# ImIntheMiddle/EmLoco

Measured on AMD Instinct MI355X. Metric: env-steps/sec (SMPL humanoid, num_envs), higher is better.
Workload: dtype f32

## Files before the change

### emloco_amd/csrc/emloco_types.h

```cpp
#pragma once
#define EMLOCO_PART_WORDS 416
#include "../../include/emloco_sim.h"
#define EMLOCO_PART_TAG(seq, part) ((seq) * 4u + (unsigned)(part))
#define EMLOCO_ERR_PART_TIMEOUT 1u

#define EMLOCO_TOPO_PARENT 0
#define EMLOCO_TOPO_DEPTH 24
#define EMLOCO_TOPO_CHILD 48
#define EMLOCO_TOPO_PDPACK 120
#define EMLOCO_TOPO_CAND 144
#define EMLOCO_TOPO_SCPAIR 240
#define EMLOCO_TOPO_WORDS 560

#define EMLOCO_MB_DYN 0
#define EMLOCO_MB_GEO 384
#define EMLOCO_MB_CAP 576
#define EMLOCO_MB_DRV 832
#define EMLOCO_MODEL_WORDS 1112

struct EmlocoSimDev {
    int n_env, n_cand, max_depth, sc_n;
    int sc_nseg;
    const int *topo;
    const float *model;
// ... 7 lines not shown
    const unsigned char *hf_mv;
    long long *prof;
    const long long *step_skip;
    const int *step_ids;
    int n_slots;
    const int *step_order;
    unsigned *step_ticks;
    int n_parts; unsigned part_seq;
    float *part_state;
    unsigned *part_flag;
    unsigned *err;
    int part_spin_max;
    int part_poison;
    unsigned long long *step_start;
};
```

### emloco_amd/csrc/sim_capi.hip

```cpp
#include <hip/hip_runtime.h>
#include <cstdlib>
#include <cstdio>
#include <cstring>
#include <string>
#include <vector>
#ifdef EMLOCO_SIM_PAIR
#include "sim_pair_kernels.hip"
#define EMLOCO_SIM_ENVS_PER_WG 2
#else
#include "sim_kernels.hip"
#define EMLOCO_SIM_ENVS_PER_WG 1
#endif
#include "topology.h"
#include "model_pack.h"
#include "sim_state.h"

namespace {

thread_local std::string g_err;

int fail(int code, const char *what, hipError_t e = hipSuccess) {
    char buf[512];
    if (e != hipSuccess) snprintf(buf, sizeof(buf), "%s: %s", what, hipGetErrorString(e));
    else snprintf(buf, sizeof(buf), "%s", what);
// ... 276 lines not shown
    if (!s || !dev_forces) return fail(EMLOCO_E_ARG, "emloco_sim_set_dof_actuation_force: null argument");
    if (!s->prepared) return fail(EMLOCO_E_STATE, "emloco_sim_set_dof_actuation_force: sim not prepared");
    if (dev_forces != s->d_tgt.p)
        HIPCHK(hipMemcpyAsync(s->d_tgt.p, dev_forces, (size_t)s->n_env * EMLOCO_NDOF * 4, hipMemcpyDeviceToDevice, (hipStream_t)stream));
    s->prm.drive_mode = 1;
    return EMLOCO_OK;
}

static int launch_order(EmlocoSim *s, hipStream_t st) {
    if (s->order_ready) { s->order_ready = false; return EMLOCO_OK; }
    hipLaunchKernelGGL(emloco::sim_order_kernel, dim3(1), dim3(1024), 0, st, s->d_ticks.p, s->n_env, s->d_order.p, s->d_order_ws.p);
    HIPCHK(hipGetLastError());
    return EMLOCO_OK;
}

int emloco_sim_step(EmlocoSim *s, int n_calls, void *stream) {
    if (!s) return fail(EMLOCO_E_ARG, "emloco_sim_step: null sim");
    if (!s->prepared) return fail(EMLOCO_E_STATE, "emloco_sim_step: sim not prepared");
    if (n_calls < 1) return fail(EMLOCO_E_ARG, "emloco_sim_step: n_calls < 1");
    if (const int rc = check_device_error(s, "emloco_sim_step")) return rc;
    EmlocoSimParams p = s->prm;
    p.n_sub = s->prm.n_sub * n_calls;
    hipStream_t st = (hipStream_t)stream;
    EmlocoSimDev d = s->dev;
    if (s->cost_order) {
        const int rc = launch_order(s, st);
        if (rc != EMLOCO_OK) return rc;
        d.step_order = s->d_order.p;
        d.step_ticks = s->d_ticks.p;
    }
    const int slot = s->ev_head;
    const bool timed = s->timing && (s->launch_no++ % s->timing_stride) == 0;
    if (timed) HIPCHK(hipEventRecord(s->ev0[slot], st));
    d.n_parts = s->n_parts < p.n_sub ? s->n_parts : p.n_sub;
    d.part_seq = ++s->part_seq; d.part_state = s->d_part_state.p; d.part_flag = s->d_part_flag.p;
    d.part_spin_max = s->part_spin_max; d.part_poison = s->part_poison;
    d.n_slots = s->n_env;
    const unsigned grid = (unsigned)(((s->n_env + EMLOCO_SIM_ENVS_PER_WG - 1) / EMLOCO_SIM_ENVS_PER_WG) * d.n_parts);
    if (d.hf) hipLaunchKernelGGL(emloco::sim_step_kernel<1>, dim3(grid), dim3(64), (size_t)s->lds_pad, st, p, d);
    else hipLaunchKernelGGL(emloco::sim_step_kernel<0>, dim3(grid), dim3(64), (size_t)s->lds_pad, st, p, d);
    HIPCHK(hipGetLastError());
    if (timed) {
        HIPCHK(hipEventRecord(s->ev1[slot], st));
        s->ev_head = (slot + 1) % EmlocoSim::kRing;
        if (s->ev_count < EmlocoSim::kRing) ++s->ev_count;
    }
    return EMLOCO_OK;
}

int emloco_sim_step_subset(EmlocoSim *s, int n_calls, const int64_t *dev_skip, const int32_t *dev_ids, int n_ids, void *stream) {
    if (!s) return fail(EMLOCO_E_ARG, "emloco_sim_step_subset: null sim");
    if (!s->prepared) return fail(EMLOCO_E_STATE, "emloco_sim_step_subset: sim not prepared");
    if (n_calls < 1) return fail(EMLOCO_E_ARG, "emloco_sim_step_subset: n_calls < 1");
    if ((dev_skip == nullptr) == (dev_ids == nullptr)) return fail(EMLOCO_E_ARG, "emloco_sim_step_subset: exactly one of skip flags / id list");
    if (dev_ids && (n_ids < 0 || n_ids > s->n_env)) return fail(EMLOCO_E_ARG, "emloco_sim_step_subset: bad id count");
    if (dev_ids && n_ids == 0) return EMLOCO_OK;
    if (const int rc = check_device_error(s, "emloco_sim_step_subset")) return rc;
    EmlocoSimParams p = s->prm;
    p.n_sub = s->prm.n_sub * n_calls;
    EmlocoSimDev d = s->dev;
    d.step_skip = (const long long *)dev_skip;
    d.step_ids = (const int *)dev_ids;
    hipStream_t st = (hipStream_t)stream;
    if (s->cost_order) {
        d.step_ticks = s->d_ticks.p;
        if (dev_skip) {
            const int rc = launch_order(s, st);
            if (rc != EMLOCO_OK) return rc;
            d.step_order = s->d_order.p;
        }
    }
    const bool timed = s->timing && dev_skip && (s->launch_no++ % s->timing_stride) == 0;
    const int slot = s->ev_head;
    if (timed) HIPCHK(hipEventRecord(s->ev0[slot], st));
    d.n_parts = dev_ids ? 1 : (s->n_parts < p.n_sub ? s->n_parts : p.n_sub);
    d.part_seq = ++s->part_seq; d.part_state = s->d_part_state.p; d.part_flag = s->d_part_flag.p;
    d.part_spin_max = s->part_spin_max; d.part_poison = s->part_poison;
    d.n_slots = dev_ids ? n_ids : s->n_env;
    const unsigned grid = (unsigned)(((d.n_slots + EMLOCO_SIM_ENVS_PER_WG - 1) / EMLOCO_SIM_ENVS_PER_WG) * d.n_parts);
    if (d.hf) hipLaunchKernelGGL(emloco::sim_step_kernel<1>, dim3(grid), dim3(64), (size_t)s->lds_pad, st, p, d);
    else hipLaunchKernelGGL(emloco::sim_step_kernel<0>, dim3(grid), dim3(64), (size_t)s->lds_pad, st, p, d);
    HIPCHK(hipGetLastError());
    if (timed) {
        HIPCHK(hipEventRecord(s->ev1[slot], st));
        s->ev_head = (slot + 1) % EmlocoSim::kRing;
        if (s->ev_count < EmlocoSim::kRing) ++s->ev_count;
    }
    return EMLOCO_OK;
}

int emloco_sim_set_split(EmlocoSim *s, int n_parts) {
    if (!s) return fail(EMLOCO_E_ARG, "emloco_sim_set_split: null sim");
    if (!s->prepared) return fail(EMLOCO_E_STATE, "emloco_sim_set_split: sim not prepared");
    if (n_parts < 1 || n_parts > 4) return fail(EMLOCO_E_ARG, "emloco_sim_set_split: 1 to 4 parts");
    if (n_parts > 1 && !s->d_part_state.p) {
        HIPCHK(hipSetDevice(s->device));
// ... 149 lines not shown
```

### emloco_amd/csrc/sim_kernels.hip

```cpp
#include <hip/hip_runtime.h>
#include "dev_math.h"
#include "sim_math.h"
#define cross3 fcross3
#define dot3 fdot3
#define dot6 fdot6
#define qmul fqmul
#define qnormalize fqnormalize
#define q2mat fq2mat
#define matvec3 fmatvec3
#define rotvec2quat frotvec2quat
#define quat2rotvec fquat2rotvec
#include "emloco_types.h"
#include "fk_device.h"
#include "order_device.h"

namespace emloco {

#define NB EMLOCO_NB
#define NDOF EMLOCO_NDOF
#define MAXC EMLOCO_MAXC
#define MAXR (3 * EMLOCO_MAXC)
#define MAXCAND EMLOCO_MAXCAND
#define EMLOCO_WH_MAX 1.0f
#define YLEN 30
// ... 197 lines not shown
                        if (dist > 1.0e-6f) { const float id_ = 1.0f / dist; for (int k = 0; k < 3; ++k) nsel[k] = dv[k] * id_; }
                        else for (int k = 0; k < 3; ++k) nsel[k] = fn[k] * ifn;
                    }
                } else if (side < 0.0f && face) {
                    const float dw = side * ifn;
                    if (dw > dsel) { dsel = dw; for (int k = 0; k < 3; ++k) nsel[k] = fn[k] * ifn; }
                }
            }
        }
    }
}

#ifndef EMLOCO_SIM_WAVES_PER_SIMD
#define EMLOCO_SIM_WAVES_PER_SIMD 3
#endif
template <int HF>
__device__ __forceinline__ void sim_step_env(const EmlocoSimParams &prm, const EmlocoSimDev &d, const int env, int &work, const int part, const int n_parts) {
    int lane = threadIdx.x;
    work = 0;

    enum { O_ROOT = 0, O_P = 16, O_V0 = 24, O_L = 36, O_PD = 48, O_R = O_PD + NB, O_W = O_R + NB * 12,
           O_L0 = O_W + NB * 24, O_CB = O_L0 + 44, O_CX = O_CB + MAXC / 4 + 3, O_CDIST = O_CX + 3 * MAXC, O_LAM = O_CDIST + MAXC,
           O_SLOT = O_LAM + MAXR, O_CRANGE = O_SLOT + 32, O_IA = O_CRANGE + 2 * NB / 4, O_G = O_IA + 180,
           O_PA = O_IA + NB * 24, O_A_ = O_PA + NB * 8, O_V = O_A_ + NB * 8,
           O_VF = O_V + NB * 8, O_AACC = O_VF + NB * 8, O_FEXT = O_AACC + NB * 8, O_PQ = O_FEXT + NB * 8,
           LDS_WORDS = (O_PQ + NB * 8 > O_G + MAXR * (MAXR + 1) / 2) ? O_PQ + NB * 8 : O_G + MAXR * (MAXR + 1) / 2 };
    static_assert(O_R % 4 == 0 && O_W % 4 == 0 && O_IA % 4 == 0 && O_PA % 4 == 0 && O_PQ % 4 == 0, "rows must be 16-byte aligned");
    static_assert(O_V - O_G >= EMLOCO_SC_MAXSEG * 8 + EMLOCO_SC_MAXHITS * 8 + 256, "limb-limb scratch does not fit its overlay");
    static_assert(LDS_WORDS * 4 <= 13312, "LDS per env above 160 KiB / 12 in 512-byte granules (three waves per SIMD, 12 envs per CU)");
    __shared__ __attribute__((aligned(16))) float lds[LDS_WORDS];
    float *sh_root = lds + O_ROOT;
    float *sh_V0 = lds + O_V0;
    float *sh_P = lds + O_P;
    float *sh_L = lds + O_L;
    int *sh_pd = (int *)(lds + O_PD);
    float (*sh_R)[12] = (float (*)[12])(lds + O_R);
    float (*sh_W)[24] = (float (*)[24])(lds + O_W);
    float *sh_L0 = lds + O_L0, *sh_L0i = lds + O_L0 + 36;
    unsigned char *sh_cbody = (unsigned char *)(lds + O_CB);
    float (*sh_cx)[3] = (float (*)[3])(lds + O_CX);
    float *sh_cdist = lds + O_CDIST;
    float *sh_lam = lds + O_LAM;
    signed char *sh_crange = (signed char *)(lds + O_CRANGE);
    unsigned char *sh_slot = (unsigned char *)(lds + O_SLOT);
// ... 19 lines not shown
    float *cf_env = d.contact_force + (size_t)env * NB * 3;
    float *lws_env = d.lambda_ws + (size_t)env * MAXCAND * 3;
    if (lane < NB) sh_pd[lane] = topo[EMLOCO_TOPO_PDPACK + lane];
    sh_slot[lane] = 255; sh_slot[lane + 64] = 255;

    const int sub_lo = (prm.n_sub * part) / n_parts, sub_hi = (prm.n_sub * (part + 1)) / n_parts;
    float *pst = d.part_state ? d.part_state + (long)env * EMLOCO_PART_WORDS : nullptr;
    float qj[4] = {0, 0, 0, 1}, wj[3] = {0, 0, 0}, edof[3] = {0, 0, 0};
    if (part == 0) {
        if ((lane < NB) && lane >= 1) {
            const float *ds = dofs_env + jdof * 2;
            float e[3] = {ds[0], ds[2], ds[4]};
            rotvec2quat(e, qj);
            wj[0] = ds[1]; wj[1] = ds[3]; wj[2] = ds[5];
            quat2rotvec(qj, edof);
        }
        if (lane == 0) {
            const float *rs = d.root_state + (long)env * 13;
            float q0[4] = {rs[3], rs[4], rs[5], rs[6]};
            qnormalize(q0);
            for (int k = 0; k < 3; ++k) { sh_root[k] = rs[k]; sh_root[7 + k] = rs[10 + k]; sh_root[10 + k] = rs[7 + k]; }
            for (int k = 0; k < 4; ++k) sh_root[3 + k] = q0[k];
        }
    } else {
        if (lane == 0) {
            int spins = 0;
            const unsigned want = EMLOCO_PART_TAG(d.part_seq, part - 1);
            while (part_flag_get(d.part_flag + env) != want && ++spins < d.part_spin_max) __builtin_amdgcn_s_sleep(16);
            sh_V0[0] = spins < d.part_spin_max ? 1.0f : 0.0f;
            if (spins >= d.part_spin_max) part_err_raise(d.err, EMLOCO_ERR_PART_TIMEOUT);
// ... 316 lines not shown
                    const int bi = sh_hitb[hh * 2], bj = sh_hitb[hh * 2 + 1];
                    if (bi == lane) for (int k = 0; k < 6; ++k) fe[k] += sh_hitw[hh * 6 + k];
                    else if (bj == lane) for (int k = 0; k < 6; ++k) fe[k] -= sh_hitw[hh * 6 + k];
                }
                for (int k = 0; k < 6; ++k) sh_fext[lane][k] = fe[k];
            }
            __syncthreads();
        }

        PSTAMP(1);
        if ((lane < NB)) {
            for (int k = 0; k < 3; ++k) {
                float dr[4];
                ld4(mdl, o_drv + 4 * k, dr);
                const float kp = lane >= 1 ? dr[0] : 0.0f, kd = lane >= 1 ? dr[1] : 0.0f;
                const float arm = lane >= 1 ? dr[2] : 0.0f, tgt = lane >= 1 ? tgt_env[jdof + k] : 0.0f;
                const float e = tgt - edof[k];
                if (prm.drive_mode == 1) {
                    const float eff = lane >= 1 ? dr[3] : 0.0f;
                    sat[k] = 2; tau[k] = tgt > eff ? eff : (tgt < -eff ? -eff : tgt); dd[k] = arm;
                } else {
                    sat[k] = 0; tau[k] = kp * e - (kd + h * kp) * wj[k]; dd[k] = arm + h * kd + h * h * kp;
                }
            }
        }

        PSTAMP(2);
#if defined(EMLOCO_DUMMY_VALU) || defined(EMLOCO_DUMMY_LDS) || defined(EMLOCO_DUMMY_SALU)
        {
#ifdef EMLOCO_DUMMY_VALU
            float z0 = h, z1 = h + 1.0f, z2 = h + 2.0f, z3 = h + 3.0f;
// ... 642 lines not shown
                    cross3(arm, ip, t);
                }
                for (int k = 0; k < 3; ++k) tq[k] = wave_sum(t[k]);
            }
            if (lane == 0) for (int k = 0; k < 3; ++k) sh_L[k] = (sh_L[4 + k] + tq[k]) * damp;
        }
        PSTAMP(9);
        bool clamped = false;
        if ((lane < NB) && lane >= 1) {
            float wn[3];
            for (int k = 0; k < 3; ++k) {
                wn[k] = fmaf(h, qdd[k], wj[k]) + dq[k];
                if (last) {
                    float dr[4];
                    ld4(mdl, o_drv + 4 * k, dr);
                    const float kpk = dr[0], kdk = dr[1], tgk = tgt_env[jdof + k];
                    const float effk = dr[3];
                    float tq = sat[k] == 0 ? kpk * (tgk - edof[k] - h * wn[k]) - kdk * wn[k]
                             : (sat[k] == 2 ? tgk : (sat[k] > 0 ? effk : -effk));
                    tq = tq > effk ? effk : (tq < -effk ? -effk : tq);
                    d.dof_force[(size_t)env * NDOF + jdof + k] = tq;
                }
                wj[k] = wn[k] * damp;
            }
            const float nj = sqrtf(dot3(wj, wj));
            if (nj > prm.max_ang_vel) { const float sc = prm.max_ang_vel / nj; wj[0] *= sc; wj[1] *= sc; wj[2] *= sc; clamped = true; }
            float e[3] = {h * wj[0], h * wj[1], h * wj[2]}, dqt[4], qn[4];
            rotvec2quat(e, dqt);
            qmul(qj, dqt, qn); qnormalize(qn);
            for (int k = 0; k < 4; ++k) qj[k] = qn[k];
            quat2rotvec(qj, edof);
// ... 52 lines not shown
            for (int k = 0; k < 3; ++k) { ds[2 * k] = edof[k]; ds[2 * k + 1] = wj[k]; }
        }
    }
    if (lane == 0) {
        float *rs = d.root_state + (long)env * 13;
        for (int k = 0; k < 3; ++k) { rs[k] = sh_root[k]; rs[7 + k] = sh_root[10 + k]; rs[10 + k] = sh_root[7 + k]; }
        for (int k = 0; k < 4; ++k) rs[3 + k] = sh_root[3 + k];
    }
    for (int s = 0; s < 2; ++s) {
        const int c = lane + 64 * s;
        if (c < MAXCAND) {
            const int os = sh_slot[c];
            for (int k = 0; k < 3; ++k) lws_env[c * 3 + k] = os != 255 ? sh_lam[3 * os + k] : 0.0f;
        }
    }
}
#undef o_dyn
#undef jdof
#undef o_drv

template <int HF>
__global__ void __attribute__((amdgpu_flat_work_group_size(64, 64), amdgpu_waves_per_eu(EMLOCO_SIM_WAVES_PER_SIMD, EMLOCO_SIM_WAVES_PER_SIMD)))
sim_step_kernel(EmlocoSimParams prm, EmlocoSimDev d) {
    const int n_parts = d.n_parts > 1 ? d.n_parts : 1;
    const int part = (int)blockIdx.x / d.n_env, slot = (int)blockIdx.x - part * d.n_env;
    if (part >= n_parts) return;
    int env = d.step_order ? d.step_order[slot] : slot;
    if (d.step_ids) { env = d.step_ids[slot]; if (env < 0) return; }
    if (d.step_skip && d.step_skip[env] != 0) return;
    env = __builtin_amdgcn_readfirstlane(env);
    const long long t0 = d.step_start ? (long long)wall_clock64() : 0ll;
    int work;
    sim_step_env<HF>(prm, d, env, work, part, n_parts);
    if (d.step_ticks && threadIdx.x == 0 && part == n_parts - 1) {
#ifdef EMLOCO_COST_KEY_TICKS
        d.step_ticks[env] = (unsigned)(((long long)wall_clock64() - t0) >> 9);
#else
        d.step_ticks[env] = (unsigned)work;
#endif
        if (d.step_start) { d.step_start[env] = (unsigned long long)t0; d.step_start[d.n_env + env] = (unsigned long long)wall_clock64(); }
    }
}

__global__ void __launch_bounds__(1024)
sim_order_kernel(const unsigned *ticks, int n, int *order, unsigned char *bucket_ws) {
    order_sort(ticks, n, order, bucket_ws);
}

// ... 24 lines not shown
```

### emloco_amd/csrc/sim_state.h

```cpp
#pragma once
#include <hip/hip_runtime.h>
#include <vector>
#include "emloco_types.h"
#include "topology.h"

template <class T> struct DevBuf {
    T *p = nullptr; size_t n = 0;
    hipError_t alloc(size_t count) { n = count; return hipMalloc((void **)&p, count * sizeof(T)); }
    hipError_t upload(const T *src, size_t count) {
        hipError_t e = alloc(count);
        if (e != hipSuccess) return e;
        return hipMemcpy(p, src, count * sizeof(T), hipMemcpyHostToDevice);
    }
    void release() { if (p) (void)hipFree(p); p = nullptr; n = 0; }
};


struct EmlocoSim {
    int device = 0;
    EmlocoSimParams prm{};
    bool have_model = false, prepared = false, timing = false;
    int n_env = 0;
    emloco::Topology topo;
    std::vector<float> h_off, h_mass, h_com, h_inertia, h_ga, h_gb, h_gr, h_kp, h_kd, h_arm, h_eff;
// ... 5 lines not shown
    std::vector<uint8_t> h_hf_mv;
    int hf_nx = 0, hf_ny = 0;
    float hf_hs = 0.0f, hf_vs = 0.0f, hf_ox = 0.0f, hf_oy = 0.0f;
    DevBuf<short> d_hf;
    DevBuf<unsigned char> d_hf_mv;
    DevBuf<int> d_topo;
    DevBuf<float> d_model;
    DevBuf<float> d_root, d_dof, d_tgt, d_rb, d_cf, d_df, d_lws;
    EmlocoSimDev dev{};
    int n_parts = 1;
    unsigned part_seq = 0;
    DevBuf<float> d_part_state;
    DevBuf<unsigned> d_part_flag;
    unsigned *h_err = nullptr;
    int part_spin_max = 1 << 22, part_poison = -1;
    int lds_pad = 0;
    bool cost_order = false;
    bool order_ready = false;
    DevBuf<unsigned> d_ticks;
    DevBuf<int> d_order;
    DevBuf<unsigned char> d_order_ws;
    static constexpr int kRing = 1024;
    std::vector<hipEvent_t> ev0, ev1;
    int ev_head = 0, ev_count = 0;
    int timing_stride = 1, launch_no = 0;
    float last_ms = -1.0f;
};
```

### emloco_amd/csrc/task_device.h

```cpp
#pragma once
#include <hip/hip_runtime.h>
#include "dev_math.h"
#include "../../include/emloco_task.h"
#include "locoval_returns_device.h"

namespace emloco {

#define TNB 24
#define TNDOF 69

__device__ __forceinline__ float linspace_f(double lo, double hi, int n, int i) {
    if (i == n - 1) return (float)hi;
    const double step = (hi - lo) / (double)(n - 1);
    return (float)(lo + (double)i * step);
}

__device__ __forceinline__ void calc_pos(const float *verts, float time, float traj_dur, float *out) {
    float phase = time / traj_dur;
    if (phase < 0.0f) phase = 0.0f;
    if (phase > 1.0f) phase = 1.0f;
    const float seg_idx = phase * (float)(EMLOCO_TRAJ_VERTS - 1);
    const long i0 = (long)floorf(seg_idx);
    const long i1 = (long)ceilf(seg_idx);
    const float lerp = seg_idx - (float)i0;
// ... 97 lines not shown
        float dlt[3], t3[3];
        for (int k = 0; k < 3; ++k) dlt[k] = key_pos[lane * 3 + k] - root_pos[k];
        ref_quat_rotate(hinv, dlt, t3);
        for (int k = 0; k < 3; ++k) out[12 + nj * 6 + n_sub + lane * 3 + k] = t3[k];
    }
    if (lane < 11) out[12 + nj * 6 + n_sub + 12 + lane] = betas[lane];
}

#ifdef EMLOCO_POST_PROFILE
__device__ long long *g_post_prof = nullptr;
#define PPSTAMP(i) do { if (g_post_prof && lane == 0 && env == t.n_env - 1) g_post_prof[i] = wall_clock64(); } while (0)
#else
#define PPSTAMP(i) do { } while (0)
#endif
#define POST_SM_FLOATS (TNB * 13 + EMLOCO_TRAJ_SAMPLES * 3 + 12 + TNB * 3 + 2 * EMLOCO_SELF_OBS + 12)
__device__ __forceinline__ void post_physics_env(const EmlocoTaskBufs &t, int mode, int env, int lane, float *sm,
                                                 const EmlocoLocoValStep *lv = nullptr, const uint8_t *lv_inverted = nullptr) {
    PPSTAMP(0);
    float (*sh_body)[13] = (float (*)[13])sm;
    float (*sh_samp)[3] = (float (*)[3])(sm + TNB * 13);
    float *sh_center = sm + TNB * 13 + EMLOCO_TRAJ_SAMPLES * 3;
    float (*sh_cf)[3] = (float (*)[3])(sh_center + 12);
    float *sh_obs = sh_center + 12 + TNB * 3, *sh_fobs = sh_obs + EMLOCO_SELF_OBS;
    float (*sh_key)[3] = (float (*)[3])(sh_fobs + EMLOCO_SELF_OBS);

    int64_t prog = t.progress_buf[env];
    if (mode & EMLOCO_POST_ADVANCE) prog += 1;
    if (lane < TNB) {
        const float *src = t.rb_state + ((long)env * TNB + lane) * 13;
        for (int k = 0; k < 13; ++k) sh_body[lane][k] = src[k];
        if (mode & EMLOCO_POST_RESET)
            for (int k = 0; k < 3; ++k) sh_cf[lane][k] = t.contact_force[((long)env * TNB + lane) * 3 + k];
// ... 109 lines not shown
            sx += masked ? 0.0f : sh_cf[bb][0];
            sy += masked ? 0.0f : sh_cf[bb][1];
            sz += masked ? 0.0f : sh_cf[bb][2];
        }
        const float ax = fabsf(sx), ay = fabsf(sy), az = fabsf(sz);
        const float mag = sqrtf(ax * ax + ay * ay + az * az);
        const bool fallen = (mag > 50.0f) && (prog > 1);
        const float dx = tar[0] - root[0], dy = tar[1] - root[1];
        const float d2 = dx * dx + dy * dy;
        const bool far = d2 > t.fail_dist * t.fail_dist;
        const int64_t term = (fallen || far) ? 1 : 0;
        t.terminate_buf[env] = term;
        done_now = ((float)prog >= t.max_episode_length - 1.0f) ? 1 : (int)term;
        t.reset_buf[env] = done_now;
    }
    if (lv && (mode & EMLOCO_POST_REWARD) && (mode & EMLOCO_POST_RESET))
        locoval_returns_env(*lv, env, lane, rew_now, 0.0f, done_now != 0, lv_inverted && lv_inverted[env]);
    if (mode & EMLOCO_POST_AMP_DONE_ONLY) {
        done_now = (mode & EMLOCO_POST_RESET) ? __shfl(done_now, 0) : (int)(t.reset_buf[env] != 0);
        if (!done_now) return;
    }

    if (mode & (EMLOCO_POST_AMP_SHIFT | EMLOCO_POST_AMP_ROW)) {
        float *amp = t.amp_obs_buf + (long)env * EMLOCO_AMP_STEPS * EMLOCO_AMP_ROW;
        if ((mode & EMLOCO_POST_AMP_SHIFT) && !t.amp_ring) {
            constexpr int NEL = (EMLOCO_AMP_STEPS - 1) * EMLOCO_AMP_ROW;
            constexpr int PER = (NEL + 63) / 64;
            float keep[PER];
            for (int j = 0; j < PER; ++j) { const int e = lane + 64 * j; keep[j] = e < NEL ? amp[e] : 0.0f; }
            __syncthreads();
            for (int j = 0; j < PER; ++j) { const int e = lane + 64 * j; if (e < NEL) amp[EMLOCO_AMP_ROW + e] = keep[j]; }
        }
        PPSTAMP(6);
        if (mode & EMLOCO_POST_AMP_ROW) {
            if (lane < 4) for (int k = 0; k < 3; ++k) sh_key[lane][k] = sh_body[t.key_bodies[lane]][k];
            __syncthreads();
            const float *ds = t.dof_state + (long)env * TNDOF * 2;
            amp_row(lane, root, root + 3, root + 7, root + 10, ds, ds + 1, 2, &sh_key[0][0], t.betas + (long)env * 17, t.dof_subset, t.n_dof_subset,
                    amp + EMLOCO_AMP_PHYS_ROW(t.amp_ring, 0) * EMLOCO_AMP_ROW);
        }
// ... 6 lines not shown
```

### emloco_amd/env/tasks/humanoid.py

```python
import numpy as np
import torch

from ... import _lib as L
from ...gym import gymapi, gymtorch
from ...gym.torch_utils import get_axis_params, to_torch
from ...model import smpl_humanoid
from ...post_physics import BODY_NAMES, LEFT_TO_RIGHT, PostPhysics, dof_subset_indices
from ...utils.flags import flags
from .base_task import BaseTask

ENABLE_MAX_COORD_OBS = True


class Humanoid(BaseTask):
    def __init__(self, cfg, sim_params, physics_engine, device_type, device_id, headless):
        self.cfg = cfg
        self.sim_params = sim_params
        self.physics_engine = physics_engine
        self.has_task = getattr(self, "has_task", False)
        self.device_type, self.device_id = device_type, device_id
        self.device = "cpu"
        if device_type == "cuda" or device_type == "GPU":
            self.device = "cuda" + ":" + str(device_id)
        self.load_smpl_configs(cfg)
# ... 314 lines not shown
        self.gym.refresh_net_contact_force_tensor(self.sim)
        return

    def pre_physics_step(self, actions):
        self.wait_obs()
        if getattr(self, "_actions_buf", None) is None or self._actions_buf.shape != actions.shape:
            self._actions_buf = torch.empty(actions.shape, dtype=torch.float32, device=self.device)
        if not self._pd_control:
            self._actions_buf.copy_(actions)
            self.actions = self._actions_buf
            forces = self.actions * self.motor_efforts.unsqueeze(0) * self.power_scale
            if not self.gym.set_dof_actuation_force_tensor(self.sim, gymtorch.unwrap_tensor(forces.contiguous())):
                raise RuntimeError("set_dof_actuation_force_tensor failed (simulator not prepared, or a tensor of the wrong shape / dtype)")
            return
        src = actions.to(device=self.device, dtype=torch.float32).contiguous()
        self._post.pd_targets(src, self._pd_action_offset, self._pd_action_scale, self._pd_zero_mask, self._pd_targets,
                              actions_copy=self._actions_buf)
        self.actions = self._actions_buf
        if not self.gym.set_dof_position_target_tensor(self.sim, gymtorch.unwrap_tensor(self._pd_targets)):
            raise RuntimeError("set_dof_position_target_tensor failed (simulator not prepared, or a tensor of the wrong shape / dtype)")
        return

    def _action_to_pd_targets(self, action):
        return self._pd_action_offset + self._pd_action_scale * action

    def _post_mode_step(self):
        return L.POST_ADVANCE | L.POST_OBS | L.POST_REWARD | L.POST_RESET

    _returns_hook = None
    _returns_in_flags = False

    def attach_returns(self, step_struct, before=None):
        self._returns_hook = step_struct
        self._returns_before = before if step_struct is not None else None

    def _launch_post(self, mode, env_ids=None):
# ... 27 lines not shown
        self._ev_flags, self._ev_obs = torch.cuda.Event(), torch.cuda.Event()

    def wait_obs(self):
        if self._obs_deferred:
            mode, self._obs_deferred = self._obs_deferred, 0
            self._launch_post(mode | L.POST_SKIP_DONE)
        if getattr(self, "_obs_pending", False):
            torch.cuda.current_stream(self.device).wait_event(self._ev_obs)
            self._obs_pending = False

    def post_physics_step(self):
        self._refresh_sim_tensors()
        mode = self._post_mode_step()
        if self.fused_chain and torch.device(self.device).type == "cuda" and getattr(self, "_fused_reset", False):
            self.wait_obs()
            if self.fused_amp_early:
                side_mode = mode & L.POST_OBS
                self._launch_post(mode & ~side_mode)
            else:
                side_mode = mode & (L.POST_OBS | L.POST_AMP_SHIFT | L.POST_AMP_ROW)
                amp = mode & (L.POST_AMP_SHIFT | L.POST_AMP_ROW)
                self._launch_post((mode & ~side_mode) | (amp | L.POST_AMP_DONE_ONLY if amp else 0))
            self._obs_deferred = side_mode
        elif self.overlap_obs and torch.device(self.device).type == "cuda":
            if getattr(self, "_obs_stream", None) is None:
                self._make_obs_stream()
            self.wait_obs()
            side_mode = mode & (L.POST_OBS | L.POST_AMP_SHIFT | L.POST_AMP_ROW)
            amp = mode & (L.POST_AMP_SHIFT | L.POST_AMP_ROW)
            self._launch_post((mode & ~side_mode) | (amp | L.POST_AMP_DONE_ONLY if amp else 0))
            main = torch.cuda.current_stream(self.device)
            self._ev_flags.record(main)
            self._obs_stream.wait_event(self._ev_flags)
            with torch.cuda.stream(self._obs_stream):
                self._launch_post(side_mode | L.POST_SKIP_DONE)
                self._ev_obs.record(self._obs_stream)
            self._obs_pending = True
# ... 18 lines not shown
```

### emloco_amd/env/tasks/humanoid_amp.py

```python
from enum import Enum

import numpy as np
import torch

from ... import _lib as L
from ...gym import gymtorch
from ...gym.torch_utils import quat_apply
from ...utils.flags import flags
from ...utils.motion_lib_synthetic import MotionLibSynthetic
from .humanoid import Humanoid


class HumanoidAMP(Humanoid):
    class StateInit(Enum):
        Default = 0
        Start = 1
        Random = 2
        Hybrid = 3

    def __init__(self, cfg, sim_params, physics_engine, device_type, device_id, headless):
        state_init = cfg["env"]["stateInit"]
        self._state_init = HumanoidAMP.StateInit[state_init]
        self._hybrid_init_prob = cfg["env"]["hybridInitProb"]
        self._num_amp_obs_steps = cfg["env"]["numAMPObsSteps"]
# ... 70 lines not shown
            rad.append(pool[id(a)][1])
        self._cand_body = torch.tensor(pool[id(self.humanoid_assets[0])][2], dtype=torch.long, device=self.device)
        self._cand_points = torch.from_numpy(np.stack(pts)).to(self.device)
        self._cand_radius = torch.from_numpy(np.stack(rad)).to(self.device)

    def _lowest_point(self, env_ids):
        pos = self._rigid_body_pos[env_ids][:, self._cand_body]
        rot = self._rigid_body_rot[env_ids][:, self._cand_body]
        wp = quat_apply(rot, self._cand_points[env_ids]) + pos
        return (wp[..., 2] - self._cand_radius[env_ids]).min(dim=-1).values

    def _post_mode_step(self):
        return super()._post_mode_step() | L.POST_AMP_SHIFT | L.POST_AMP_ROW

    def post_physics_step(self):
        if self.amp_ring:
            self._amp_head = (self._amp_head + self._num_amp_obs_steps - 1) % self._num_amp_obs_steps
            self._amp_ring_to_bufs()
        super().post_physics_step()
        self.extras["amp_obs"] = None if self.amp_ring else self._amp_obs_buf.view(-1, self.get_num_amp_obs())
        return

    amp_ring = False
    _amp_head = 0

    def enable_amp_ring(self, on=True):
        on = bool(on)
        if on == self.amp_ring:
            return
        if on and (torch.device(self.device).type != "cuda" or not getattr(self, "_fused_reset", False)):
            raise RuntimeError("amp ring: needs the fused device step / reset kernels (a CUDA device, fused_reset)")
        if hasattr(self, "wait_obs"):
            self.wait_obs()
        if not on:
            self._amp_obs_buf.copy_(self.amp_obs_logical().view_as(self._amp_obs_buf))
        self._amp_head = 0
        self.amp_ring = on
        self._amp_ring_to_bufs()
        if not on:
# ... 161 lines not shown
```

### emloco_amd/sim.py

```python
import ctypes as C

import numpy as np
import torch

from . import _lib as L
from .model import HumanoidModel, pack_models

_TORCH_TYPESTR = {torch.float32: "<f4", torch.int32: "<i4", torch.int64: "<i8", torch.uint8: "|u1", torch.int16: "<i2"}


class _DevView:

    def __init__(self, ptr, shape, dtype, owner):
        self.__cuda_array_interface__ = {"shape": tuple(int(s) for s in shape), "typestr": _TORCH_TYPESTR[dtype],
                                         "data": (int(ptr), False), "version": 2, "strides": None}
        self._owner = owner


def wrap_device_pointer(ptr, shape, dtype, device, owner=None):
    return torch.as_tensor(_DevView(ptr, shape, dtype, owner), device=device)


def current_stream_handle(device):
    return C.c_void_p(torch.cuda.current_stream(device).cuda_stream)
# ... 74 lines not shown

    def _stream(self):
        return current_stream_handle(self.device)

    def set_pd_targets(self, targets):
        L.check(self.lib.emloco_sim_set_pd_targets(self._h, dptr(targets), self._stream()), "emloco_sim_set_pd_targets")

    def set_dof_actuation_force(self, forces):
        if forces.dtype != torch.float32 or forces.numel() != self.num_envs * 69:
            raise L.EmlocoError("actuation forces must be a float32 [n_env][69] tensor")
        L.check(self.lib.emloco_sim_set_dof_actuation_force(self._h, dptr(forces), self._stream()), "emloco_sim_set_dof_actuation_force")

    def step(self, n_calls=1):
        L.check(self.lib.emloco_sim_step(self._h, int(n_calls), self._stream()), "emloco_sim_step")

    def set_cost_order(self, on=True):
        L.check(self.lib.emloco_sim_set_cost_order(self._h, int(bool(on))), "emloco_sim_set_cost_order")

    def set_split(self, n_parts=2):
        L.check(self.lib.emloco_sim_set_split(self._h, int(n_parts)), "emloco_sim_set_split")

    def step_subset(self, n_calls=1, skip=None, ids=None):
        if skip is not None:
            assert skip.dtype == torch.int64 and skip.numel() == self.num_envs
        if ids is not None:
            assert ids.dtype == torch.int32
        L.check(self.lib.emloco_sim_step_subset(self._h, int(n_calls), dptr(skip), dptr(ids), 0 if ids is None else int(ids.numel()),
                                                self._stream()), "emloco_sim_step_subset")

    def sync(self):
# ... 48 lines not shown
```

### include/emloco_sim.h

```cpp
#ifndef EMLOCO_SIM_H
#define EMLOCO_SIM_H
#include <stdint.h>

#ifdef __cplusplus
extern "C" {
#endif

#define EMLOCO_NB 24
#define EMLOCO_NDOF 69
#define EMLOCO_MAXC 20
#define EMLOCO_MAXCAND 96

enum { EMLOCO_GEOM_SPHERE = 0, EMLOCO_GEOM_CAPSULE = 1, EMLOCO_GEOM_BOX = 2 };

enum {
    EMLOCO_OK = 0,
    EMLOCO_E_ARG = -1,
    EMLOCO_E_HIP = -2,
    EMLOCO_E_STATE = -3,
    EMLOCO_E_NODEV = -4
};

typedef struct {
    int32_t n_sub;
// ... 62 lines not shown
int emloco_sim_create(const EmlocoSimParams *params, int device, EmlocoSim **out);
int emloco_sim_destroy(EmlocoSim *sim);
int emloco_sim_set_models(EmlocoSim *sim, const EmlocoModelDesc *desc);
int emloco_sim_set_self_collision(EmlocoSim *sim, const EmlocoSelfCollisionDesc *desc);
int emloco_sim_set_ground_heightfield(EmlocoSim *sim, const int16_t *samples, int nx, int ny, float horizontal_scale,
                                      float vertical_scale, float origin_x, float origin_y);
int emloco_sim_set_ground_mesh_moves(EmlocoSim *sim, const int8_t *move_x, const int8_t *move_y);
int emloco_sim_prepare(EmlocoSim *sim);
int emloco_sim_get_params(EmlocoSim *sim, EmlocoSimParams *out);
int emloco_sim_set_params(EmlocoSim *sim, const EmlocoSimParams *in);
int emloco_sim_tensor(EmlocoSim *sim, int kind, void **dev_ptr, int64_t shape[2]);
int emloco_sim_set_pd_targets(EmlocoSim *sim, const float *dev_targets, void *stream);
int emloco_sim_set_dof_actuation_force(EmlocoSim *sim, const float *dev_forces, void *stream);
int emloco_sim_step(EmlocoSim *sim, int n_calls, void *stream);
int emloco_sim_step_subset(EmlocoSim *sim, int n_calls, const int64_t *dev_skip, const int32_t *dev_env_ids, int n_ids, void *stream);
int emloco_sim_set_split(EmlocoSim *sim, int n_parts);
int emloco_sim_set_cost_order(EmlocoSim *sim, int on);
int emloco_sim_sync(EmlocoSim *sim, void *stream);
int emloco_sim_debug_poison_part(EmlocoSim *sim, int env, int spin_max);
int emloco_sim_fk_indexed(EmlocoSim *sim, const int32_t *dev_env_ids, int n, void *stream);
int emloco_sim_cost_ticks(EmlocoSim *sim, unsigned *host_ticks, unsigned long long *host_start, int n);
int emloco_sim_profile(EmlocoSim *sim, long long *host_out, int n);
int emloco_sim_set_root_state_indexed(EmlocoSim *sim, const float *dev_full, const int32_t *dev_env_ids, int n, void *stream);
int emloco_sim_set_dof_state_indexed(EmlocoSim *sim, const float *dev_full, const int32_t *dev_env_ids, int n, void *stream);
int emloco_sim_refresh_bodies(EmlocoSim *sim, void *stream);
int emloco_sim_num_candidates(EmlocoSim *sim);
float emloco_sim_last_step_ms(EmlocoSim *sim);
int emloco_sim_enable_timing(EmlocoSim *sim, int on);
int emloco_sim_timing_stats(EmlocoSim *sim, int *n_launches, float *total_ms);

// ... 5 lines not shown
```

Before: 9.263 million.

## Fuse PD-target computation and post-physics flags pass into the sim step kernel

Adds an epilogue to the rigid-body step kernel that runs the task's post-physics pass (progress, reward, reset flags, AMP ring row, LocoVal returns) for each env right after physics. It also computes PD targets from raw actions inside the kernel instead of in a separate launch. Python arms these per step through new C API calls, and falls back to the old launches when conditions are not met. This removes two kernel launches and a round trip of state through global memory per step. In exchange the sim kernel gets more registers and code, and a one-shot arming protocol that must not be interrupted by another launch.

```diff
diff --git a/emloco_amd/csrc/emloco_types.h b/emloco_amd/csrc/emloco_types.h
--- a/emloco_amd/csrc/emloco_types.h
+++ b/emloco_amd/csrc/emloco_types.h
@@ -1,6 +1,8 @@
 #pragma once
 #define EMLOCO_PART_WORDS 416
 #include "../../include/emloco_sim.h"
+#include "../../include/emloco_task.h"
+#include "../../include/emloco_predictor.h"
 #define EMLOCO_PART_TAG(seq, part) ((seq) * 4u + (unsigned)(part))
 #define EMLOCO_ERR_PART_TIMEOUT 1u
 
@@ -45,3 +47,26 @@
     int part_poison;
     unsigned long long *step_start;
 };
+
+struct EmlocoSimPost {
+    int mode;
+    int has_lv;
+    const uint8_t *inverted;
+    EmlocoTaskBufs t;
+    EmlocoLocoValStep lv;
+    const float *actions, *pd_offset, *pd_scale;
+    const uint8_t *pd_zero_mask;
+    float *actions_copy, *pd_target;
+};
+
+struct EmlocoSimPostArm {
+    EmlocoSimPost post{};
+    int ran = 0;
+    EmlocoSimPost take(int drive_mode, const void *skip, const void *ids) {
+        EmlocoSimPost p = post;
+        post = EmlocoSimPost{};
+        if (drive_mode != 0 || skip || ids) p = EmlocoSimPost{};
+        ran = (p.mode ? 1 : 0) | (p.actions ? 2 : 0);
+        return p;
+    }
+};
diff --git a/emloco_amd/csrc/sim_capi.hip b/emloco_amd/csrc/sim_capi.hip
--- a/emloco_amd/csrc/sim_capi.hip
+++ b/emloco_amd/csrc/sim_capi.hip
@@ -314,11 +314,72 @@
     return EMLOCO_OK;
 }
 
+int emloco_sim_attach_post(EmlocoSim *s, const void *task_bufs, int mode, const void *lv_step, const uint8_t *inverted) {
+    if (!s) return fail(EMLOCO_E_ARG, "emloco_sim_attach_post: null sim");
+    s->arm.post.mode = 0; s->arm.post.has_lv = 0;
+    if (!task_bufs || mode == 0) return EMLOCO_OK;
+#ifdef EMLOCO_SIM_PAIR
+    return fail(EMLOCO_E_STATE, "emloco_sim_attach_post: the two-envs-per-wave build has no epilogue");
+#else
+    if (!s->prepared) return fail(EMLOCO_E_STATE, "emloco_sim_attach_post: sim not prepared");
+    const EmlocoTaskBufs &t = *(const EmlocoTaskBufs *)task_bufs;
+    const EmlocoLocoValStep *lv = (const EmlocoLocoValStep *)lv_step;
+    if (mode & ~EMLOCO_SIM_POST_BITS)
+        return fail(EMLOCO_E_ARG, "emloco_sim_attach_post: the epilogue carries progress, reward, reset flags and the AMP row only (no observations, no SKIP_DONE)");
+    if (t.n_env != s->n_env || t.rb_state != s->d_rb.p || t.dof_state != s->d_dof.p || t.dof_force != s->d_df.p || t.contact_force != s->d_cf.p)
+        return fail(EMLOCO_E_ARG, "emloco_sim_attach_post: the task buffers must read this simulator's own state tensors, for all its envs");
+    if (!t.progress_buf || !t.traj_verts) return fail(EMLOCO_E_ARG, "emloco_sim_attach_post: missing tensors");
+    if ((mode & EMLOCO_POST_REWARD) && (!t.rew_buf || !t.reward_raw)) return fail(EMLOCO_E_ARG, "emloco_sim_attach_post: reward buffers missing");
+    if ((mode & EMLOCO_POST_RESET) && (!t.reset_buf || !t.terminate_buf || !t.contact_body_mask))
+        return fail(EMLOCO_E_ARG, "emloco_sim_attach_post: reset buffers missing");
+    if ((mode & EMLOCO_POST_AMP_DONE_ONLY) && !t.reset_buf) return fail(EMLOCO_E_ARG, "emloco_sim_attach_post: AMP_DONE_ONLY needs reset_buf");
+    if (mode & (EMLOCO_POST_AMP_ROW | EMLOCO_POST_AMP_SHIFT)) {
+        const int n_sub = t.n_dof_subset;
+        if (!t.amp_obs_buf || !t.dof_subset || !t.key_bodies || !t.betas || n_sub < 0 || n_sub % 3 != 0 || 35 + 3 * n_sub > EMLOCO_AMP_ROW)
+            return fail(EMLOCO_E_ARG, "emloco_sim_attach_post: AMP buffers missing");
+        if (!t.amp_ring) return fail(EMLOCO_E_ARG, "emloco_sim_attach_post: AMP rows ride in the epilogue in the ring layout only (EmlocoTaskBufs.amp_ring)");
+    }
+    if (lv) {
+        if (!(mode & EMLOCO_POST_REWARD) || !(mode & EMLOCO_POST_RESET))
+            return fail(EMLOCO_E_ARG, "emloco_sim_attach_post: the return bookkeeping follows the reward and the reset flag of the same launch");
+        if (lv->n_env != t.n_env || !lv->current_rewards || !lv->current_lengths || !lv->current_combined_rewards || !lv->discount_coefs ||
+            !lv->waypoint_traj || !lv->init_pose || !lv->init_vel || !lv->traj13 || !lv->pose || !lv->vel || !lv->target || !lv->weight)
+            return fail(EMLOCO_E_ARG, "emloco_sim_attach_post: LocoVal step buffers missing or for another env count");
+        if ((lv->staged_reward == nullptr) != (lv->staged_done == nullptr))
+            return fail(EMLOCO_E_ARG, "emloco_sim_attach_post: staged_reward and staged_done go together");
+        s->arm.post.lv = *lv; s->arm.post.has_lv = 1;
+    }
+    s->arm.post.t = t; s->arm.post.inverted = inverted; s->arm.post.mode = mode;
+    return EMLOCO_OK;
+#endif
+}
+
+int emloco_sim_attach_pd_targets(EmlocoSim *s, const float *actions, const float *offset, const float *scale, const uint8_t *zero_mask,
+                                 float *actions_copy) {
+    if (!s) return fail(EMLOCO_E_ARG, "emloco_sim_attach_pd_targets: null sim");
+    s->arm.post.actions = nullptr;
+    if (!actions) return EMLOCO_OK;
+#ifdef EMLOCO_SIM_PAIR
+    return fail(EMLOCO_E_STATE, "emloco_sim_attach_pd_targets: not in the two-envs-per-wave build");
+#else
+    if (!s->prepared) return fail(EMLOCO_E_STATE, "emloco_sim_attach_pd_targets: sim not prepared");
+    if (!offset || !scale || !zero_mask) return fail(EMLOCO_E_ARG, "emloco_sim_attach_pd_targets: null argument");
+    if (actions == s->d_tgt.p || actions_copy == s->d_tgt.p) return fail(EMLOCO_E_ARG, "emloco_sim_attach_pd_targets: the actions must not alias the target tensor");
+    s->arm.post.actions = actions; s->arm.post.pd_offset = offset; s->arm.post.pd_scale = scale; s->arm.post.pd_zero_mask = zero_mask;
+    s->arm.post.actions_copy = actions_copy == actions ? nullptr : actions_copy;
+    s->arm.post.pd_target = s->d_tgt.p;
+    return EMLOCO_OK;
+#endif
+}
+
+int emloco_sim_post_ran(EmlocoSim *s) { return s ? s->arm.ran : 0; }
+
 int emloco_sim_step(EmlocoSim *s, int n_calls, void *stream) {
     if (!s) return fail(EMLOCO_E_ARG, "emloco_sim_step: null sim");
+    const EmlocoSimPost post = s->arm.take(s->prm.drive_mode, nullptr, nullptr);
     if (!s->prepared) return fail(EMLOCO_E_STATE, "emloco_sim_step: sim not prepared");
     if (n_calls < 1) return fail(EMLOCO_E_ARG, "emloco_sim_step: n_calls < 1");
-    if (const int rc = check_device_error(s, "emloco_sim_step")) return rc;
+    if (const int rc = check_device_error(s, "emloco_sim_step")) { s->arm.ran = 0; return rc; }
     EmlocoSimParams p = s->prm;
     p.n_sub = s->prm.n_sub * n_calls;
     hipStream_t st = (hipStream_t)stream;
@@ -337,8 +398,13 @@
     d.part_spin_max = s->part_spin_max; d.part_poison = s->part_poison;
     d.n_slots = s->n_env;
     const unsigned grid = (unsigned)(((s->n_env + EMLOCO_SIM_ENVS_PER_WG - 1) / EMLOCO_SIM_ENVS_PER_WG) * d.n_parts);
+#ifdef EMLOCO_SIM_PAIR
     if (d.hf) hipLaunchKernelGGL(emloco::sim_step_kernel<1>, dim3(grid), dim3(64), (size_t)s->lds_pad, st, p, d);
     else hipLaunchKernelGGL(emloco::sim_step_kernel<0>, dim3(grid), dim3(64), (size_t)s->lds_pad, st, p, d);
+#else
+    if (d.hf) hipLaunchKernelGGL(emloco::sim_step_kernel<1>, dim3(grid), dim3(64), (size_t)s->lds_pad, st, p, d, post);
+    else hipLaunchKernelGGL(emloco::sim_step_kernel<0>, dim3(grid), dim3(64), (size_t)s->lds_pad, st, p, d, post);
+#endif
     HIPCHK(hipGetLastError());
     if (timed) {
         HIPCHK(hipEventRecord(s->ev1[slot], st));
@@ -354,6 +420,7 @@
     if (n_calls < 1) return fail(EMLOCO_E_ARG, "emloco_sim_step_subset: n_calls < 1");
     if ((dev_skip == nullptr) == (dev_ids == nullptr)) return fail(EMLOCO_E_ARG, "emloco_sim_step_subset: exactly one of skip flags / id list");
     if (dev_ids && (n_ids < 0 || n_ids > s->n_env)) return fail(EMLOCO_E_ARG, "emloco_sim_step_subset: bad id count");
+    (void)s->arm.take(s->prm.drive_mode, dev_skip, dev_ids);
     if (dev_ids && n_ids == 0) return EMLOCO_OK;
     if (const int rc = check_device_error(s, "emloco_sim_step_subset")) return rc;
     EmlocoSimParams p = s->prm;
@@ -378,8 +445,13 @@
     d.part_spin_max = s->part_spin_max; d.part_poison = s->part_poison;
     d.n_slots = dev_ids ? n_ids : s->n_env;
     const unsigned grid = (unsigned)(((d.n_slots + EMLOCO_SIM_ENVS_PER_WG - 1) / EMLOCO_SIM_ENVS_PER_WG) * d.n_parts);
+#ifdef EMLOCO_SIM_PAIR
     if (d.hf) hipLaunchKernelGGL(emloco::sim_step_kernel<1>, dim3(grid), dim3(64), (size_t)s->lds_pad, st, p, d);
     else hipLaunchKernelGGL(emloco::sim_step_kernel<0>, dim3(grid), dim3(64), (size_t)s->lds_pad, st, p, d);
+#else
+    if (d.hf) hipLaunchKernelGGL(emloco::sim_step_kernel<1>, dim3(grid), dim3(64), (size_t)s->lds_pad, st, p, d, EmlocoSimPost{});
+    else hipLaunchKernelGGL(emloco::sim_step_kernel<0>, dim3(grid), dim3(64), (size_t)s->lds_pad, st, p, d, EmlocoSimPost{});
+#endif
     HIPCHK(hipGetLastError());
     if (timed) {
         HIPCHK(hipEventRecord(s->ev1[slot], st));
diff --git a/emloco_amd/csrc/sim_kernels.hip b/emloco_amd/csrc/sim_kernels.hip
--- a/emloco_amd/csrc/sim_kernels.hip
+++ b/emloco_amd/csrc/sim_kernels.hip
@@ -1,5 +1,6 @@
 #include <hip/hip_runtime.h>
 #include "dev_math.h"
+#include "task_device.h"
 #include "sim_math.h"
 #define cross3 fcross3
 #define dot3 fdot3
@@ -235,8 +236,17 @@
 #ifndef EMLOCO_SIM_WAVES_PER_SIMD
 #define EMLOCO_SIM_WAVES_PER_SIMD 3
 #endif
+__device__ __forceinline__ float pd_target_of(const EmlocoSimPost &post, const float *tgt_env, int env, int dd) {
+    if (post.actions) {
+        const float a = post.actions[(size_t)env * NDOF + dd];
+        return post.pd_zero_mask[dd] ? 0.0f : post.pd_offset[dd] + post.pd_scale[dd] * a;
+    }
+    return tgt_env[dd];
+}
+#define EMLOCO_SIM_POST_BITS (EMLOCO_POST_ADVANCE | EMLOCO_POST_REWARD | EMLOCO_POST_RESET | EMLOCO_POST_AMP_ROW | EMLOCO_POST_AMP_SHIFT | EMLOCO_POST_AMP_DONE_ONLY)
+
 template <int HF>
-__device__ __forceinline__ void sim_step_env(const EmlocoSimParams &prm, const EmlocoSimDev &d, const int env, int &work, const int part, const int n_parts) {
+__device__ __forceinline__ void sim_step_env(const EmlocoSimParams &prm, const EmlocoSimDev &d, const EmlocoSimPost &post, const int env, int &work, const int part, const int n_parts) {
     int lane = threadIdx.x;
     work = 0;
 
@@ -249,6 +259,7 @@
     static_assert(O_R % 4 == 0 && O_W % 4 == 0 && O_IA % 4 == 0 && O_PA % 4 == 0 && O_PQ % 4 == 0, "rows must be 16-byte aligned");
     static_assert(O_V - O_G >= EMLOCO_SC_MAXSEG * 8 + EMLOCO_SC_MAXHITS * 8 + 256, "limb-limb scratch does not fit its overlay");
     static_assert(LDS_WORDS * 4 <= 13312, "LDS per env above 160 KiB / 12 in 512-byte granules (three waves per SIMD, 12 envs per CU)");
+    static_assert(POST_SM_FLOATS <= LDS_WORDS, "the epilogue's workspace overlays the blob");
     __shared__ __attribute__((aligned(16))) float lds[LDS_WORDS];
     float *sh_root = lds + O_ROOT;
     float *sh_V0 = lds + O_V0;
@@ -298,6 +309,13 @@
             rotvec2quat(e, qj);
             wj[0] = ds[1]; wj[1] = ds[3]; wj[2] = ds[5];
             quat2rotvec(qj, edof);
+            if (post.actions) {
+                for (int k = 0; k < 3; ++k) {
+                    const size_t i = (size_t)env * NDOF + jdof + k;
+                    if (post.actions_copy) post.actions_copy[i] = post.actions[i];
+                    post.pd_target[i] = pd_target_of(post, tgt_env, env, jdof + k);
+                }
+            }
         }
         if (lane == 0) {
             const float *rs = d.root_state + (long)env * 13;
@@ -644,7 +662,7 @@
                 float dr[4];
                 ld4(mdl, o_drv + 4 * k, dr);
                 const float kp = lane >= 1 ? dr[0] : 0.0f, kd = lane >= 1 ? dr[1] : 0.0f;
-                const float arm = lane >= 1 ? dr[2] : 0.0f, tgt = lane >= 1 ? tgt_env[jdof + k] : 0.0f;
+                const float arm = lane >= 1 ? dr[2] : 0.0f, tgt = lane >= 1 ? pd_target_of(post, tgt_env, env, jdof + k) : 0.0f;
                 const float e = tgt - edof[k];
                 if (prm.drive_mode == 1) {
                     const float eff = lane >= 1 ? dr[3] : 0.0f;
@@ -1317,7 +1335,7 @@
                 if (last) {
                     float dr[4];
                     ld4(mdl, o_drv + 4 * k, dr);
-                    const float kpk = dr[0], kdk = dr[1], tgk = tgt_env[jdof + k];
+                    const float kpk = dr[0], kdk = dr[1], tgk = pd_target_of(post, tgt_env, env, jdof + k);
                     const float effk = dr[3];
                     float tq = sat[k] == 0 ? kpk * (tgk - edof[k] - h * wn[k]) - kdk * wn[k]
                              : (sat[k] == 2 ? tgk : (sat[k] > 0 ? effk : -effk));
@@ -1400,6 +1418,10 @@
             for (int k = 0; k < 3; ++k) lws_env[c * 3 + k] = os != 255 ? sh_lam[3 * os + k] : 0.0f;
         }
     }
+    if (post.mode) {
+        __syncthreads();
+        post_physics_env<EMLOCO_SIM_POST_BITS, true>(post.t, post.mode, env, lane, lds, &post.lv, post.inverted, post.has_lv != 0);
+    }
 }
 #undef o_dyn
 #undef jdof
@@ -1407,7 +1429,7 @@
 
 template <int HF>
 __global__ void __attribute__((amdgpu_flat_work_group_size(64, 64), amdgpu_waves_per_eu(EMLOCO_SIM_WAVES_PER_SIMD, EMLOCO_SIM_WAVES_PER_SIMD)))
-sim_step_kernel(EmlocoSimParams prm, EmlocoSimDev d) {
+sim_step_kernel(EmlocoSimParams prm, EmlocoSimDev d, EmlocoSimPost post = EmlocoSimPost{}) {
     const int n_parts = d.n_parts > 1 ? d.n_parts : 1;
     const int part = (int)blockIdx.x / d.n_env, slot = (int)blockIdx.x - part * d.n_env;
     if (part >= n_parts) return;
@@ -1417,7 +1439,7 @@
     env = __builtin_amdgcn_readfirstlane(env);
     const long long t0 = d.step_start ? (long long)wall_clock64() : 0ll;
     int work;
-    sim_step_env<HF>(prm, d, env, work, part, n_parts);
+    sim_step_env<HF>(prm, d, post, env, work, part, n_parts);
     if (d.step_ticks && threadIdx.x == 0 && part == n_parts - 1) {
 #ifdef EMLOCO_COST_KEY_TICKS
         d.step_ticks[env] = (unsigned)(((long long)wall_clock64() - t0) >> 9);
diff --git a/emloco_amd/csrc/sim_state.h b/emloco_amd/csrc/sim_state.h
--- a/emloco_amd/csrc/sim_state.h
+++ b/emloco_amd/csrc/sim_state.h
@@ -43,6 +43,7 @@
     DevBuf<unsigned> d_part_flag;
     unsigned *h_err = nullptr;
     int part_spin_max = 1 << 22, part_poison = -1;
+    EmlocoSimPostArm arm;
     int lds_pad = 0;
     bool cost_order = false;
     bool order_ready = false;
diff --git a/emloco_amd/csrc/task_device.h b/emloco_amd/csrc/task_device.h
--- a/emloco_amd/csrc/task_device.h
+++ b/emloco_amd/csrc/task_device.h
@@ -135,8 +135,10 @@
 #define PPSTAMP(i) do { } while (0)
 #endif
 #define POST_SM_FLOATS (TNB * 13 + EMLOCO_TRAJ_SAMPLES * 3 + 12 + TNB * 3 + 2 * EMLOCO_SELF_OBS + 12)
+template <int ALLOWED = -1, bool RING_ONLY = false>
 __device__ __forceinline__ void post_physics_env(const EmlocoTaskBufs &t, int mode, int env, int lane, float *sm,
-                                                 const EmlocoLocoValStep *lv = nullptr, const uint8_t *lv_inverted = nullptr) {
+                                                 const EmlocoLocoValStep *lv = nullptr, const uint8_t *lv_inverted = nullptr, bool lv_on = true) {
+    mode &= ALLOWED;
     PPSTAMP(0);
     float (*sh_body)[13] = (float (*)[13])sm;
     float (*sh_samp)[3] = (float (*)[3])(sm + TNB * 13);
@@ -276,7 +278,7 @@
         done_now = ((float)prog >= t.max_episode_length - 1.0f) ? 1 : (int)term;
         t.reset_buf[env] = done_now;
     }
-    if (lv && (mode & EMLOCO_POST_REWARD) && (mode & EMLOCO_POST_RESET))
+    if (lv && lv_on && (mode & EMLOCO_POST_REWARD) && (mode & EMLOCO_POST_RESET))
         locoval_returns_env(*lv, env, lane, rew_now, 0.0f, done_now != 0, lv_inverted && lv_inverted[env]);
     if (mode & EMLOCO_POST_AMP_DONE_ONLY) {
         done_now = (mode & EMLOCO_POST_RESET) ? __shfl(done_now, 0) : (int)(t.reset_buf[env] != 0);
@@ -285,7 +287,7 @@
 
     if (mode & (EMLOCO_POST_AMP_SHIFT | EMLOCO_POST_AMP_ROW)) {
         float *amp = t.amp_obs_buf + (long)env * EMLOCO_AMP_STEPS * EMLOCO_AMP_ROW;
-        if ((mode & EMLOCO_POST_AMP_SHIFT) && !t.amp_ring) {
+        if (!RING_ONLY && (mode & EMLOCO_POST_AMP_SHIFT) && !t.amp_ring) {
             constexpr int NEL = (EMLOCO_AMP_STEPS - 1) * EMLOCO_AMP_ROW;
             constexpr int PER = (NEL + 63) / 64;
             float keep[PER];
diff --git a/emloco_amd/env/tasks/humanoid.py b/emloco_amd/env/tasks/humanoid.py
--- a/emloco_amd/env/tasks/humanoid.py
+++ b/emloco_amd/env/tasks/humanoid.py
@@ -1,3 +1,5 @@
+import os
+
 import numpy as np
 import torch
 
@@ -352,12 +354,57 @@
                 raise RuntimeError("set_dof_actuation_force_tensor failed (simulator not prepared, or a tensor of the wrong shape / dtype)")
             return
         src = actions.to(device=self.device, dtype=torch.float32).contiguous()
-        self._post.pd_targets(src, self._pd_action_offset, self._pd_action_scale, self._pd_zero_mask, self._pd_targets,
-                              actions_copy=self._actions_buf)
+        self._post_armed = self._arm_sim_post(src)
+        if not self._post_armed:
+            self._post.pd_targets(src, self._pd_action_offset, self._pd_action_scale, self._pd_zero_mask, self._pd_targets,
+                                  actions_copy=self._actions_buf)
         self.actions = self._actions_buf
         if not self.gym.set_dof_position_target_tensor(self.sim, gymtorch.unwrap_tensor(self._pd_targets)):
             raise RuntimeError("set_dof_position_target_tensor failed (simulator not prepared, or a tensor of the wrong shape / dtype)")
         return
+
+    _post_armed = False
+
+    def _flags_mode_fused(self, mode):
+        side_mode = mode & (L.POST_OBS | L.POST_AMP_SHIFT | L.POST_AMP_ROW)
+        amp = mode & (L.POST_AMP_SHIFT | L.POST_AMP_ROW)
+        return (mode & ~side_mode) | (amp | L.POST_AMP_DONE_ONLY if amp else 0), side_mode
+
+    def _arm_sim_post(self, actions):
+        native = getattr(self.sim, "native", None)
+        if (native is None or os.environ.get("EMLOCO_SIM_POST", "1") == "0" or not self.fused_chain or self.fused_amp_early
+                or torch.device(self.device).type != "cuda" or not getattr(self, "_fused_reset", False)
+                or self.paused or not self.enable_viewer_sync or getattr(self, "_rs_pending", False)):
+            return False
+        flags_mode, _ = self._flags_mode_fused(self._post_mode_step())
+        if (flags_mode & (L.POST_AMP_SHIFT | L.POST_AMP_ROW)) and not getattr(self, "amp_ring", False):
+            return False
+        if self._post_bufs is None:
+            self._ensure_post_bufs()
+        if hasattr(self, "_advance_amp_ring"):
+            self._advance_amp_ring()
+        hook, inv = self._returns_hook, None
+        if hook is not None:
+            if getattr(self, "_returns_before", None) is not None:
+                self._returns_before()
+            inv = self.inverted if isinstance(getattr(self, "inverted", None), torch.Tensor) else None
+            if inv is not None and inv.dtype == torch.bool:
+                inv = inv.view(torch.uint8)
+            inv = inv.contiguous() if inv is not None else None
+        native.attach_post(self._post_bufs, flags_mode, hook, inv)
+        if os.environ.get("EMLOCO_SIM_POST_PD", "1") != "0":
+            native.attach_pd_targets(actions, self._pd_action_offset, self._pd_action_scale, self._pd_zero_mask, self._actions_buf)
+        else:
+            self._post.pd_targets(actions, self._pd_action_offset, self._pd_action_scale, self._pd_zero_mask, self._pd_targets,
+                                  actions_copy=self._actions_buf)
+        self._armed_keep = (actions, inv)
+        return True
+
+    def _ensure_post_bufs(self):
+        self._post_bufs = self._make_post_bufs()
+        if hasattr(self, "_amp_ring_to_bufs"):
+            self._amp_ring_to_bufs()
+        return self._post_bufs
 
     def _action_to_pd_targets(self, action):
         return self._pd_action_offset + self._pd_action_scale * action
@@ -415,13 +462,19 @@
         mode = self._post_mode_step()
         if self.fused_chain and torch.device(self.device).type == "cuda" and getattr(self, "_fused_reset", False):
             self.wait_obs()
-            if self.fused_amp_early:
+            if self._post_armed:
+                self._post_armed = False
+                if not (self.sim.native.post_ran() & 1):
+                    raise RuntimeError("the rigid-body launch did not run the flags pass it was armed with (another launch came between)")
+                _, side_mode = self._flags_mode_fused(mode)
+                if self._returns_hook is not None:
+                    self._returns_in_flags = True
+            elif self.fused_amp_early:
                 side_mode = mode & L.POST_OBS
                 self._launch_post(mode & ~side_mode)
             else:
-                side_mode = mode & (L.POST_OBS | L.POST_AMP_SHIFT | L.POST_AMP_ROW)
-                amp = mode & (L.POST_AMP_SHIFT | L.POST_AMP_ROW)
-                self._launch_post((mode & ~side_mode) | (amp | L.POST_AMP_DONE_ONLY if amp else 0))
+                flags_mode, side_mode = self._flags_mode_fused(mode)
+                self._launch_post(flags_mode)
             self._obs_deferred = side_mode
         elif self.overlap_obs and torch.device(self.device).type == "cuda":
             if getattr(self, "_obs_stream", None) is None:
diff --git a/emloco_amd/env/tasks/humanoid_amp.py b/emloco_amd/env/tasks/humanoid_amp.py
--- a/emloco_amd/env/tasks/humanoid_amp.py
+++ b/emloco_amd/env/tasks/humanoid_amp.py
@@ -108,15 +108,19 @@
         return super()._post_mode_step() | L.POST_AMP_SHIFT | L.POST_AMP_ROW
 
     def post_physics_step(self):
+        if not self._post_armed:
+            self._advance_amp_ring()
+        super().post_physics_step()
+        self.extras["amp_obs"] = None if self.amp_ring else self._amp_obs_buf.view(-1, self.get_num_amp_obs())
+        return
+
+    amp_ring = False
+    _amp_head = 0
+
+    def _advance_amp_ring(self):
         if self.amp_ring:
             self._amp_head = (self._amp_head + self._num_amp_obs_steps - 1) % self._num_amp_obs_steps
             self._amp_ring_to_bufs()
-        super().post_physics_step()
-        self.extras["amp_obs"] = None if self.amp_ring else self._amp_obs_buf.view(-1, self.get_num_amp_obs())
-        return
-
-    amp_ring = False
-    _amp_head = 0
 
     def enable_amp_ring(self, on=True):
         on = bool(on)
diff --git a/emloco_amd/sim.py b/emloco_amd/sim.py
--- a/emloco_amd/sim.py
+++ b/emloco_amd/sim.py
@@ -112,6 +112,17 @@
     def step(self, n_calls=1):
         L.check(self.lib.emloco_sim_step(self._h, int(n_calls), self._stream()), "emloco_sim_step")
 
+    def attach_post(self, task_bufs, mode, lv_step=None, inverted=None):
+        L.check(self.lib.emloco_sim_attach_post(self._h, None if task_bufs is None else C.byref(task_bufs), int(mode),
+                                                None if lv_step is None else C.byref(lv_step), dptr(inverted)), "emloco_sim_attach_post")
+
+    def attach_pd_targets(self, actions, offset=None, scale=None, zero_mask=None, actions_copy=None):
+        L.check(self.lib.emloco_sim_attach_pd_targets(self._h, dptr(actions), dptr(offset), dptr(scale), dptr(zero_mask), dptr(actions_copy)),
+                "emloco_sim_attach_pd_targets")
+
+    def post_ran(self):
+        return int(self.lib.emloco_sim_post_ran(self._h))
+
     def set_cost_order(self, on=True):
         L.check(self.lib.emloco_sim_set_cost_order(self._h, int(bool(on))), "emloco_sim_set_cost_order")
 
diff --git a/include/emloco_sim.h b/include/emloco_sim.h
--- a/include/emloco_sim.h
+++ b/include/emloco_sim.h
@@ -100,6 +100,11 @@
 int emloco_sim_set_dof_actuation_force(EmlocoSim *sim, const float *dev_forces, void *stream);
 int emloco_sim_step(EmlocoSim *sim, int n_calls, void *stream);
 int emloco_sim_step_subset(EmlocoSim *sim, int n_calls, const int64_t *dev_skip, const int32_t *dev_env_ids, int n_ids, void *stream);
+int emloco_sim_attach_post(EmlocoSim *sim, const void *task_bufs , int mode,
+                           const void *lv_step , const uint8_t *dev_inverted);
+int emloco_sim_attach_pd_targets(EmlocoSim *sim, const float *dev_actions, const float *dev_offset, const float *dev_scale,
+                                 const uint8_t *dev_zero_mask, float *dev_actions_copy);
+int emloco_sim_post_ran(EmlocoSim *sim);
 int emloco_sim_set_split(EmlocoSim *sim, int n_parts);
 int emloco_sim_set_cost_order(EmlocoSim *sim, int on);
 int emloco_sim_sync(EmlocoSim *sim, void *stream);
```

After: 9.139 million. 1.3% lower.
